# mbitsnbites/himg

Hardware: AMD Instinct MI355X
Metric: Mpixels/s encode+decode, 4K RGBA q=50 (higher is better)
Workload: dtype u8/i16/i32 integer

## Files before the change

himg_amd/csrc/himg_dev.h:

```cpp
#ifndef HIMG_DEV_H_
#define HIMG_DEV_H_

#include <hip/hip_runtime.h>
#include <stdint.h>

#include "search_step.h"

namespace himg_dev {

constexpr int kNumSym = 261;
constexpr int kHistStride = 264;
constexpr int kLresSpan = 16384;
constexpr int kIterSyms = 4096;
constexpr int kTreeStride = 384;
constexpr int kMaxCodeLen = 32;
constexpr int kHeadLen = 175;

struct Geom {
  int W, H, C, stride;
  int rows, cols, mrows, mcols;
  int chan_size, lres_size;
  int row_block;
  int ycbcr;
  int lres_spans;
  int use_blocks;
  int fix_t2;
  int lres_serial;
  int max_sub;
  int lead_bits;
  int prefetch_rows;
  int count_wave;
  int wide_q;
  int emit_rows;
  int front;
  int row_tokens;
  long long frame_bytes;
  long long fres_size;
};

struct EncWs {
  uint8_t *avg, *low;        size_t plane_stride;
  uint8_t *lres_sym;         size_t lres_stride;
  uint8_t *fres_sym;         size_t fres_stride;
  uint32_t *hist;
  uint32_t *span_hist_l;
  uint32_t *span_hist_f;
  uint32_t *lres_trail;
  uint64_t *codes;
  uint32_t *lens;
  uint8_t *tree;
  uint32_t *tree_nbytes;
  uint64_t *span_bit0;
  uint32_t *span_bits;
  int32_t *status;
  uint16_t *tok;
  uint32_t *tok_cnt;
  int tok_seg, tok_nseg, tok_cap;
};

constexpr uint32_t kTokRunMark = 0x0100u;
constexpr int kTokMaxRun = 255;
constexpr int kTokIter = 2048;
constexpr int kTokRunPiece = 16662;
constexpr int kTokStage = 1152;
inline int tok_slots_beyond(int zeros_max) { return 5 + 3 * (zeros_max / kTokRunPiece); }
inline int tok_seg_pad(int row_block) {
  const int pad = (tok_slots_beyond(row_block) + 7) & ~7;
  return pad > 64 ? pad : 64;
}
inline int tok_stage_need(int row_block, int seg) {
  const int alone = 1024 + tok_slots_beyond(row_block);
  const int carried = 7 + 1024 + tok_slots_beyond(seg < row_block ? seg : row_block);
  return alone > carried ? alone : carried;
}

struct StaticChunks {
  uint8_t head[176];
  uint8_t mid[272];
  int mid_len;
};

struct ShiftTables {
  uint8_t s[2][64];
};

struct LresTables {
  int16_t tab[128];
  uint8_t code[512];
};

struct QualTab {
// ... 228 lines not shown
```

himg_amd/csrc/himg_hip.hip:

```cpp
#include "himg_hip.h"

#include <hip/hip_runtime.h>

#include <cmath>
#include <cstdio>
#include <cstdlib>
#include <cstring>
#include <string>
#include <vector>

#include "himg_dev.h"
#include "himg_tables.h"

using namespace himg_dev;

namespace himg_dev {

struct Profiler {
  bool enabled = false;
  struct Rec { const char *name; hipEvent_t a, b; };
  std::vector<Rec> pending;
  struct Acc { std::string name; double ms = 0; int n = 0; };
  std::vector<Acc> acc;
  const char *cur = nullptr;
// ... 28 lines not shown
  hipEvent_t b;
  hipEventCreate(&b);
  hipEventRecord(b, s);
  p->pending.push_back({p->cur, p->cur_a, b});
}

}

namespace {

struct DevBuf {
  void *p = nullptr;
  size_t cap = 0;
  bool reserve(size_t n) {
    if (n <= cap) return true;
    if (p) hipFree(p);
    p = nullptr;
    cap = 0;
    if (hipMalloc(&p, n) != hipSuccess) return false;
    cap = n;
    return true;
  }
  void release() {
    if (p) hipFree(p);
    p = nullptr;
    cap = 0;
  }
};

size_t round_up(size_t x, size_t a) { return (x + a - 1) / a * a; }

struct HostResult {
  uint32_t size;
  int32_t status;
  int32_t quality;
  uint64_t sse;
};
struct PipeMeta {
  HostResult res[2];
  uint32_t dec_size[2];
};

}

struct himg_hip_ctx {
  int device = 0;
  std::string err;
  Profiler prof;
  hipStream_t last_stream = nullptr;
  HostOpts opts;
  int fix_t2 = 0;
  int max_sub = 4096;
  int lead_bits = 128;
  int lres_serial = 0;
  int prefetch_rows = 1;
  int count_wave = -1, emit_rows = -1;
  int row_tokens = -1;
  int front = -1;
  DecStreams dstr;
  hipStream_t side_enc = nullptr;
  hipEvent_t ev_fork_e = nullptr, ev_join_e = nullptr;

  DevBuf fmap_lut;
  size_t host_bytes = 0;
  struct Pipe {
    bool ready = false;
    hipStream_t s_in = nullptr, s_comp = nullptr, s_out = nullptr;
    hipEvent_t ev_in[2] = {nullptr, nullptr}, ev_k[2] = {nullptr, nullptr}, ev_out[2] = {nullptr, nullptr};
    DevBuf in[2], out[2], meta[2];
    PipeMeta *h_meta = nullptr;
  } pipe;

  DevBuf e_planes, e_lres, e_fres, e_small, e_spanhist, e_tok, e_tokx;
  DevBuf e_qtab, e_search;
  DevBuf e_stab, e_rec;
  bool qtab_ready = false;
  Geom enc_geom{};
  EncWs enc_ws{};
  int enc_batch = 0;
  bool enc_valid = false;

  DevBuf d_frames, d_nodes, d_grp, d_gyc, d_sub, d_lane, d_rows, d_lres, d_fres, d_planes, d_sizes, d_stats, d_spec;
  Geom dec_geom{};
  DecWs dec_ws{};
  int dec_batch = 0;
  bool dec_valid = false;
  hipEvent_t ev_range[HIMG_MAX_WALK_RANGES] = {};
  int n_ranges = 0;
  struct HeadToken {
    bool valid = false;
    int w = 0, h = 0, c = 0;
    const void *packed = nullptr;
    uint32_t size = 0;
    void *stream = nullptr;
  } head;

  DevBuf h_in, h_out, h_result, h_status, h_index;
  uint32_t *hp_index = nullptr;
  size_t hp_index_cap = 0;

  struct SizeRing {
    static constexpr int kSlots = 4;
    uint32_t *h[kSlots] = {nullptr, nullptr, nullptr, nullptr};
    size_t cap[kSlots] = {0, 0, 0, 0};
    hipEvent_t ev[kSlots] = {nullptr, nullptr, nullptr, nullptr};
    bool busy[kSlots] = {false, false, false, false};
    int next = 0;
  } sizes_ring;

  struct {
    bool valid = false;
    Geom g{};
    StaticChunks sc{};
    ShiftTables st{};
    LresTables lt{};
    int r0 = 0, r1 = 0;
  } shard;
};

static int fail(himg_hip_ctx *ctx, int code, const char *what, hipError_t e = hipSuccess) {
  if (ctx) {
    ctx->err = what;
    if (e != hipSuccess) { ctx->err += ": "; ctx->err += hipGetErrorString(e); }
  }
  return code;
}

#define HIP_TRY(ctx, expr)                                                  \
  do {                                                                      \
    hipError_t e_ = (expr);                                                 \
    if (e_ != hipSuccess) return fail(ctx, HIMG_ERR_HIP, #expr, e_);        \
  } while (0)

static bool make_geom(int width, int height, int pixel_stride, int num_channels, int use_ycbcr,
                      Geom *g) {
  if (width < 1 || height < 1 || num_channels < 1 || num_channels > 4 ||
      pixel_stride < num_channels)
    return false;
  g->W = width; g->H = height; g->C = num_channels; g->stride = pixel_stride;
  g->rows = (height + 7) >> 3; g->cols = (width + 7) >> 3;
  g->mrows = (g->rows + 15) / 16; g->mcols = (g->cols + 15) / 16;
  g->chan_size = g->mrows * g->mcols + g->rows * g->cols;
  const long long lres = (long long)g->chan_size * num_channels;
  const long long fres = (long long)g->rows * g->cols * 64 * num_channels;
  if (fres > 0x7fffffffLL || (long long)width * height * pixel_stride > 0x7fffffffLL) return false;
  g->lres_size = (int)lres;
  g->row_block = g->cols * num_channels * 64;
  g->ycbcr = (use_ycbcr && num_channels >= 3) ? 1 : 0;
  g->lres_spans = (g->lres_size + kLresSpan - 1) / kLresSpan;
  g->use_blocks = g->rows > 1 ? 1 : 0;
  g->fix_t2 = 0;
  g->max_sub = 4096;
  g->lead_bits = 128;
  g->lres_serial = 0;
  g->count_wave = g->emit_rows = g->row_tokens = g->front = -1;
  g->wide_q = 0;
  g->prefetch_rows = 1;
  g->frame_bytes = (long long)width * height * pixel_stride;
  g->fres_size = fres;
  return true;
}

static void apply_settings(const himg_hip_ctx *ctx, Geom *g) {
  g->fix_t2 = ctx->fix_t2;
  g->max_sub = ctx->max_sub;
  g->lead_bits = ctx->lead_bits;
  g->lres_serial = ctx->lres_serial;
  g->prefetch_rows = ctx->prefetch_rows;
  g->count_wave = ctx->count_wave;
  g->emit_rows = ctx->emit_rows;
  g->row_tokens = ctx->row_tokens;
  g->front = ctx->front;
}

extern "C" size_t himg_hip_max_packed_size(int width, int height, int num_channels) {
  Geom g;
  if (!make_geom(width, height, num_channels, num_channels, 1, &g)) return 0;
  size_t n = 12 + 19 + 136 + 8 + 72 + 188 + 8;
  n += (size_t)g.lres_size + kTreeStride;
  n += (size_t)g.fres_size + kTreeStride + 4u * (size_t)g.rows;
  return round_up(n + 64, 256);
}

extern "C" int himg_hip_create(int device, himg_hip_ctx **out) {
  if (!out) return HIMG_ERR_ARG;
  *out = nullptr;
  int count = 0;
  if (hipGetDeviceCount(&count) != hipSuccess || count < 1) return HIMG_ERR_HIP;
  if (device < 0 || device >= count) return HIMG_ERR_ARG;
  if (hipSetDevice(device) != hipSuccess) return HIMG_ERR_HIP;
  himg_hip_ctx *ctx = new himg_hip_ctx();
  ctx->device = device;
  HostOpts &o = ctx->opts;
  if (const char *e = std::getenv("HIMG_FORCE_UNFUSED")) o.allow_fused = !(e[0] == '1');
  if (const char *e = std::getenv("HIMG_WALK_SEGS")) o.walk_segs = atoi(e);
  if (const char *e = std::getenv("HIMG_SIDE_STREAM")) o.use_side = !(e[0] == '0');
  if (const char *e = std::getenv("HIMG_PERSIST_ROWS")) o.persist_rows = atoi(e);
  if (const char *e = std::getenv("HIMG_PREFETCH_ROWS")) ctx->prefetch_rows = atoi(e);
  if (const char *e = std::getenv("HIMG_FIX_T2")) ctx->fix_t2 = e[0] == '1';
  if (const char *e = std::getenv("HIMG_FORCE_LRES_SERIAL")) ctx->lres_serial = e[0] == '1';
  if (const char *e = std::getenv("HIMG_MAX_SUB_BITS")) {
    const int v = std::atoi(e);
    if (v >= 128 && v <= 4096 && v % 32 == 0) ctx->max_sub = v;
  }
  if (const char *e = std::getenv("HIMG_COUNT_WAVE")) ctx->count_wave = atoi(e) ? 1 : 0;
  if (const char *e = std::getenv("HIMG_EMIT_ROWS")) ctx->emit_rows = atoi(e) ? 1 : 0;
  if (const char *e = std::getenv("HIMG_ROW_TOKENS")) ctx->row_tokens = atoi(e) ? 1 : 0;
  if (const char *e = std::getenv("HIMG_FRONT")) ctx->front = atoi(e) ? 1 : 0;
  if (const char *e = std::getenv("HIMG_LEAD_BITS")) {
    const int v = std::atoi(e);
    if (v >= 0 && v <= 4096) ctx->lead_bits = v;
  }
  int n_cu = 0;
  if (hipDeviceGetAttribute(&n_cu, hipDeviceAttributeMultiprocessorCount, device) == hipSuccess && n_cu > 0) o.n_cu = n_cu;
  if (himg_dev::enc_set_kernel_attrs() != hipSuccess || himg_dev::dec_set_kernel_attrs() != hipSuccess) {
    delete ctx;
    return HIMG_ERR_HIP;
  }
  std::vector<uint8_t> lut(32769);
  int16_t fmap[128];
  himg_tables_fullres_map(fmap);
  for (int a = 0; a <= 32767; ++a) lut[a] = himg_tables_map_to_8bit(fmap, a);
  lut[32768] = (uint8_t)(0u - himg_tables_map_to_8bit(fmap, -32768));
  if (!ctx->fmap_lut.reserve(round_up(lut.size(), 256)) ||
      hipMemcpy(ctx->fmap_lut.p, lut.data(), lut.size(), hipMemcpyHostToDevice) != hipSuccess) {
    delete ctx;
    return HIMG_ERR_HIP;
  }
  int prio_least = 0, prio_greatest = 0;
  (void)hipDeviceGetStreamPriorityRange(&prio_least, &prio_greatest);
  bool ev_ok = true;
  for (int k = 0; k < kWalkSegs; ++k)
    ev_ok = ev_ok && hipEventCreateWithFlags(&ctx->dstr.ev_walk[k], hipEventDisableTiming) == hipSuccess &&
            hipEventCreateWithFlags(&ctx->dstr.ev_cnt[k], hipEventDisableTiming) == hipSuccess &&
            hipEventCreateWithFlags(&ctx->dstr.ev_win[k], hipEventDisableTiming) == hipSuccess;
  if (!ev_ok || hipStreamCreateWithPriority(&ctx->dstr.side, hipStreamNonBlocking, prio_least) != hipSuccess ||
      hipStreamCreateWithPriority(&ctx->dstr.side2, hipStreamNonBlocking, prio_least) != hipSuccess ||
      hipEventCreateWithFlags(&ctx->dstr.ev_fork, hipEventDisableTiming) != hipSuccess ||
      hipStreamCreateWithFlags(&ctx->side_enc, hipStreamNonBlocking) != hipSuccess ||
      hipEventCreateWithFlags(&ctx->ev_fork_e, hipEventDisableTiming) != hipSuccess ||
      hipEventCreateWithFlags(&ctx->ev_join_e, hipEventDisableTiming) != hipSuccess) {
    himg_hip_destroy(ctx);
    return HIMG_ERR_HIP;
  }
  ctx->dstr.side3 = ctx->side_enc;
  *out = ctx;
  return HIMG_OK;
}

extern "C" void himg_hip_destroy(himg_hip_ctx *ctx) {
  if (!ctx) return;
  hipSetDevice(ctx->device);
  hipDeviceSynchronize();
// ... 223 lines not shown
  const size_t plane = round_up((size_t)g.C * g.rows * g.cols, 256);
  const size_t lres = round_up((size_t)g.lres_size + 16, 256);
  const size_t fres = round_up((size_t)g.fres_size + 16, 256);
  if (head_only) {
    const size_t nst = 2 * (size_t)batch - 1;
    if (!ctx->d_frames.reserve(sizeof(DecFrame) * batch) || !ctx->d_nodes.reserve(nst * (2 * kNumSym) * 4) ||
        !ctx->d_grp.reserve(nst * (1u << kLutBits) * 8) || !ctx->d_gyc.reserve(nst * (1u << kLutBits) * 4) ||
        !ctx->d_sub.reserve(nst * kSubEntries * 8) || !ctx->d_lres.reserve(lres * batch) ||
        !ctx->d_planes.reserve(plane * batch) || !ctx->d_sizes.reserve((size_t)batch * 8) ||
        !ctx->d_stats.reserve(((size_t)batch * (g.rows + 1) * 8 + (size_t)batch * 4) * 4))
      return fail(ctx, HIMG_ERR_HIP, "decoder workspace allocation failed");
  } else if (!ctx->d_frames.reserve(sizeof(DecFrame) * batch) ||
      !ctx->d_nodes.reserve((size_t)batch * 2 * (2 * kNumSym) * 4) ||
      !ctx->d_grp.reserve((size_t)batch * 2 * (1u << kLutBits) * 8) ||
      !ctx->d_gyc.reserve((size_t)batch * 2 * (1u << kLutBits) * 4) ||
      !ctx->d_sub.reserve((size_t)batch * 2 * kSubEntries * 8) ||
      !ctx->d_lane.reserve((size_t)batch * g.rows * (2 * kDecThreads + himg_dev::kRecHdr + (region || himg_dev::dec_rows_fit_lds(g) ? 0 : 6 * kDecThreads)) * 4) ||
      !ctx->d_rows.reserve((size_t)batch * g.rows * 4 * 2) || !ctx->d_lres.reserve(lres * batch) ||
      (!region && !ctx->d_fres.reserve(fres * batch)) || !ctx->d_planes.reserve(plane * batch) ||
      !ctx->d_sizes.reserve((size_t)batch * 20) ||
      !ctx->d_stats.reserve(((size_t)batch * (g.rows + 1) * 8 + (size_t)batch * 4 + (size_t)batch * g.rows * 8) * 4))
    return fail(ctx, HIMG_ERR_HIP, "decoder workspace allocation failed");
  w.frames = (DecFrame *)ctx->d_frames.p;
  w.nodes = (uint32_t *)ctx->d_nodes.p;
  w.grp = (uint2 *)ctx->d_grp.p;
  w.gyc = (uint32_t *)ctx->d_gyc.p;
  w.sub = (uint2 *)ctx->d_sub.p;
  w.lane_start = head_only ? nullptr : (uint32_t *)ctx->d_lane.p;
  w.lane_off = head_only ? nullptr : w.lane_start + (size_t)batch * g.rows * kDecThreads;
  w.lane_q = (head_only || region || himg_dev::dec_rows_fit_lds(g)) ? nullptr : w.lane_off + (size_t)batch * g.rows * (kDecThreads + himg_dev::kRecHdr);
  w.row_off = head_only ? nullptr : (uint32_t *)ctx->d_rows.p;
  w.row_len = head_only ? nullptr : w.row_off + (size_t)batch * g.rows;
  w.lres_sym = (uint8_t *)ctx->d_lres.p; w.lres_stride = lres;
  w.fres_sym = (head_only || region) ? nullptr : (uint8_t *)ctx->d_fres.p; w.fres_stride = (head_only || region) ? 0 : fres;
  w.low = (uint8_t *)ctx->d_planes.p; w.plane_stride = plane;
  w.stats = (uint32_t *)ctx->d_stats.p;
  w.parse_stats = w.stats + (size_t)batch * (g.rows + 1) * 8;
  w.rc_stats = head_only ? nullptr : w.parse_stats + (size_t)batch * 4;
  {
    const size_t max_bits = 8ull * ((size_t)g.lres_size + kTreeStride);
    const size_t cb = (size_t)kDecThreads * kLresSubBits;
    int nch = (int)((max_bits + cb - 1) / cb);
    if (nch > 1024) nch = 1024;
    w.lres_chunks = nch;
    size_t off = 0;
    auto carve = [&](size_t bytes) { size_t o = off; off += round_up(bytes, 256); return o; };
    const size_t o_ss = carve((size_t)batch * nch * kDecThreads * 4);
    const size_t o_sc = carve((size_t)batch * nch * kDecThreads * 4);
    const size_t o_se = carve((size_t)batch * nch * 8);
    const size_t o_st = carve((size_t)batch * nch * 8);
    const size_t o_sp = carve((size_t)batch * nch * kDecThreads * 4);
    const size_t o_fe = carve((size_t)batch * nch * 8);
    const size_t o_vb = carve((size_t)batch * nch * 8);
    const size_t o_ok = carve((size_t)batch * 4);
    const size_t o_eb = carve((size_t)batch * 8);
    const size_t o_mm = carve((size_t)batch * nch * kDecThreads * 4 * himg_dev::kLresMemoWords);
    if (!ctx->d_spec.reserve(off)) return fail(ctx, HIMG_ERR_HIP, "decoder workspace allocation failed");
    uint8_t *b = (uint8_t *)ctx->d_spec.p;
    w.spec_start = (uint32_t *)(b + o_ss); w.spec_cnt = (uint32_t *)(b + o_sc);
    w.spec_end = (uint64_t *)(b + o_se); w.spec_tot = (uint64_t *)(b + o_st);
    w.spec_endpos = (uint32_t *)(b + o_sp); w.fix_end = (uint64_t *)(b + o_fe);
    w.ver_base = (uint64_t *)(b + o_vb); w.ver_ok = (int32_t *)(b + o_ok);
    w.lres_endbit = (uint64_t *)(b + o_eb);
    w.spec_memo = (uint32_t *)(b + o_mm);
  }
  ctx->dec_geom = g;
  ctx->dec_batch = batch;
  ctx->dec_valid = true;
  return HIMG_OK;
}

static std::string format_message(int32_t st) {
  static const char *kStage[] = {"", "Not a RIFF HIMG file.\n", "Error decoding header.\n",
                                 "Error decoding low-res mapping function.\n",
                                 "Error decoding low-res data.\n",
                                 "Error decoding quantization configuration.\n",
                                 "Error decoding full-res mapping function.\n",
                                 "Error decoding full-res data.\n"};
  std::string m;
  if (st & 0x100) m += "Error: Invalid Huffman data.\n";
  const int stage = (st >> 4) & 7;
  m += kStage[stage];
  return m;
}

static int status_to_code(int32_t st) {
  st &= 15;
  switch (st) {
    case 0: return HIMG_OK;
    case 1: return HIMG_ERR_ARG;
    case 3: return HIMG_ERR_UNSUPPORTED;
    case 4: return HIMG_ERR_FORMAT;
    case 5: return HIMG_ERR_CAPACITY;
    default: return HIMG_ERR_HIP;
  }
}

static int status_error(himg_hip_ctx *ctx, int32_t st, const char *what = "device decode reported an error") {
  const int code = status_to_code(st);
  if (code == HIMG_ERR_FORMAT) ctx->err = format_message(st);
  else fail(ctx, code, what);
  return code;
}

static int decode_args(himg_hip_ctx *ctx, int width, int height, int num_channels, int batch, DecWsKind kind,
                       const void *d_packed, const void *d_out, const size_t *in_stride, const char *bad, Geom *g) {
  if (!make_geom(width, height, num_channels, num_channels, 1, g)) return fail(ctx, HIMG_ERR_ARG, "bad geometry");
// ... 1971 lines not shown
```

himg_amd/csrc/kernels_dec.hip:

```cpp
#include "himg_dev.h"
#include "loop_counts.h"

#include <cstdlib>
#include <type_traits>

namespace himg_dev {

__device__ static constexpr uint8_t kScanD[64] = {
    0,  1,  9,  8,  16, 17, 18, 10, 2,  3,  11, 19, 27, 26, 25, 24,
    32, 33, 34, 35, 36, 28, 20, 12, 4,  5,  13, 21, 29, 37, 45, 44,
    43, 42, 41, 40, 48, 49, 50, 51, 52, 53, 54, 46, 38, 30, 22, 14,
    6,  7,  15, 23, 31, 39, 47, 55, 63, 62, 61, 60, 59, 58, 57, 56};

__device__ static constexpr uint8_t kInvScanD[64] = {
    0, 1, 8, 9, 24, 25, 48, 49, 3, 2, 7, 10, 23, 26, 47, 50, 4, 5, 6, 11, 22, 27, 46, 51, 15, 14, 13, 12, 21, 28, 45, 52, 16, 17, 18, 19, 20, 29, 44, 53, 35, 34, 33, 32, 31, 30, 43, 54, 36, 37, 38, 39, 40, 41, 42, 55, 63, 62, 61, 60, 59, 58, 57, 56};

constexpr int kStGeom = 1, kStUnsupported = 3, kStFormat = 4;
__device__ __host__ constexpr int fmt_err(int stage, int huff) { return kStFormat | (stage << 4) | (huff << 8); }
constexpr int kMaxDepth = 32;
constexpr int kMaxNodes = 2 * kNumSym - 1;
constexpr int kMaxSlow = 128;

__device__ __forceinline__ int clamp255d(int x) { return x < 0 ? 0 : (x > 255 ? 255 : x); }

// ... 1369 lines not shown
  if (end_bp != ~0u) sh->endbit = (unsigned long long)(end_bp - rel0);
  __syncthreads();
  const long long c_t1 = clock64();
  int bad = sh->err;
  if (pl.tot < out_size) bad = 1;
  const unsigned long long E = sh->endbit;
  if (!bad && !(E <= P1 && E + 8 > P1 && E > 0)) bad = 1;
  if (tid == 0 && stats) {
    stats[0] = 1; stats[1] = pl.rounds;
    stats[4] = 0; stats[5] = (uint32_t)((c_t1 - c_t0) >> 4);
    stats[6] = pay_len; stats[7] = out_size;
  }
  return bad;
}

__device__ __attribute__((noinline)) int decode_stream_fused_cold(const uint8_t *p, uint32_t stream_size,
                                                                  uint32_t pay_off, uint32_t pay_len, uint32_t out_size,
                                                                  const uint32_t *grp_lds, const uint32_t *nd_lds,
                                                                  StreamShared *sh, uint8_t *lds_out, uint32_t *stats,
                                                                  uint32_t max_sub, uint32_t lead_bits) {
  GrpTables tb;
  tb.grp = reinterpret_cast<const uint2 *>(grp_lds); tb.gx = nullptr; tb.gy = nullptr; tb.nd = nd_lds;
  return decode_stream<true, false, true>(p, stream_size, pay_off, pay_len, out_size, tb, sh, lds_out, nullptr, nullptr,
                                          stats, max_sub, lead_bits);
}

__device__ __forceinline__ void load_dec_tables(const DecWs &ws, const DecFrame *df, int f, int strm,
                                                LdsTables *T) {
  const uint32_t *nodes = ws.nodes + ((size_t)f * 2 + strm) * (kMaxNodes + 1);
  const int nn = min(df->s[strm].num_nodes, kMaxNodes + 1);
  for (int k = threadIdx.x; k < nn; k += kDecThreads) T->nd[k] = nodes[k];
  const uint4 *gg = reinterpret_cast<const uint4 *>(ws.grp + ((size_t)f * 2 + strm) * (1u << kLutBits));
  for (int k = threadIdx.x; k < (1 << kLutBits) / 2; k += kDecThreads)
    reinterpret_cast<uint4 *>(T->grp)[k] = gg[k];
  const uint4 *gs = reinterpret_cast<const uint4 *>(ws.sub + ((size_t)f * 2 + strm) * kSubEntries);
  for (int k = threadIdx.x; k < kSubEntries / 2; k += kDecThreads)
    reinterpret_cast<uint4 *>(T->grp + (1 << kLutBits))[k] = gs[k];
}

__global__ __launch_bounds__(kDecThreads) void k_dec_huff(Geom g, DecWs ws, const uint8_t *packed,
                                                          size_t in_stride, const uint32_t *sizes,
                                                          int first_block, int lres_fallback_only,
                                                          int use_row_count) {
  __shared__ uint32_t win[kWinBytes / 4 + 1];
  __shared__ LdsTables T;
  __shared__ StreamShared sh;

  const int blk = blockIdx.x + first_block, f = blockIdx.y;
  DecFrame *df = ws.frames + f;
  if (threadIdx.x == 0) sh.flag = df->status;
  __syncthreads();
  if (sh.flag) return;
  const int strm = blk == 0 ? 0 : 1;
  if (strm == 0 && lres_fallback_only && ws.ver_ok[f]) return;
  const uint8_t *p = packed + (size_t)f * in_stride;
  uint32_t pay_off, pay_len, out_size;
  uint8_t *out;
  const uint32_t *pre_start = nullptr, *pre_off = nullptr;
  if (strm == 0) {
    pay_off = df->s[0].payload_off;
    pay_len = df->s[0].chunk_end - pay_off;
    out_size = (uint32_t)g.lres_size;
    out = ws.lres_sym + (size_t)f * ws.lres_stride;
  } else {
    const int r = blk - 1;
    pay_off = ws.row_off[(size_t)f * g.rows + r];
    pay_len = ws.row_len[(size_t)f * g.rows + r];
    out_size = (uint32_t)g.row_block;
    out = ws.fres_sym + (size_t)f * ws.fres_stride + (size_t)r * g.row_block;
    if (use_row_count) {
      pre_start = ws.lane_start + ((size_t)f * g.rows + r) * kDecThreads;
      pre_off = ws.lane_off + ((size_t)f * g.rows + r) * (kDecThreads + kRecHdr);
      if (use_row_count == 2 && pre_off[kDecThreads + 2] != 0) return;
    }
  }
  load_dec_tables(ws, df, f, strm, &T);
  __syncthreads();
  const GrpTables tb = tables_of(&T);
  const int bad = decode_stream<false>(p, sizes[f], pay_off, pay_len, out_size, tb, &sh, nullptr, win,
                                       out, ws.stats + ((size_t)f * (g.rows + 1) + blk) * 8,
                                       (uint32_t)g.max_sub, (uint32_t)g.lead_bits, pre_start, pre_off);
  if (bad && threadIdx.x == 0) atomicMax(&df->status, fmt_err(strm == 0 ? 4 : 7, 1));
}

constexpr int kLresChunkBits = kDecThreads * kLresSubBits;

constexpr int kLresPayWords = kDecThreads * kLresSubBits / 32 + 8;
constexpr int kLresMemo = kLresMemoWords;
template <bool FIX>
__device__ __forceinline__ void lres_chain_body(const Geom &g, const DecWs &ws, const uint8_t *p, uint32_t stream_size,
                                const DecFrame *df, int f, int k, const GrpTables &tb, StreamShared *sh,
                                uint32_t *s_pay) {
  const int tid = threadIdx.x;
  const uint32_t pay_off = df->s[0].payload_off;
  const unsigned long long P1 = 8ull * (df->s[0].chunk_end - pay_off);
  const unsigned long long cur = (unsigned long long)k * kLresChunkBits;
  const size_t slot = (size_t)f * ws.lres_chunks + k;
  uint64_t *end_out = FIX ? ws.fix_end : ws.spec_end;
  GReader gr;
  const uint32_t rel0 = gr.attach(p, stream_size, 8ull * pay_off + cur);
  LReader rd;
  stage_payload(gr, s_pay, (uint32_t)kLresPayWords);
  __syncthreads();
  rd.w = (const __attribute__((address_space(3))) uint32_t *)s_pay;
  rd.jmax = kLresPayWords - 1;
  const unsigned long long rem = P1 - cur;
  const uint32_t rel_end = rel0 + (uint32_t)(rem < (unsigned long long)kLresChunkBits ? rem : kLresChunkBits);
// ... 24 lines not shown
      if (m != ~0u) { memo[3 * e] = my_b0 + (m & 63u); memo[3 * e + 1] = lim + ((m >> 6) & 63u); memo[3 * e + 2] = m >> 12; }
    }
  }
  const long long c_in = clock64();
  lean_fixpoint<false, LReader, kLresMemo>(rd, tb, sh, first, active, lim, &start, &endpos, &cnt, &rounds, FIX,
                                           (uint32_t)g.lead_bits, nullptr, nullptr, memo);
  const long long c_fix = clock64() - c_in;
  if (!FIX) {
#pragma unroll
    for (int e = 0; e < kLresMemo; ++e) {
      const uint32_t ds = memo[3 * e] - my_b0, de = memo[3 * e + 1] - lim;
      gm[e] = (memo[3 * e] == ~0u || tid == 0 || ds > 46u || de > 46u || memo[3 * e + 2] >= (1u << 20))
                  ? ~0u : (ds | (de << 6) | (memo[3 * e + 2] << 12));
    }
  }
  unsigned long long tot;
  block_scan_u64(cnt, sh->sm64, &tot);
  ws.spec_start[slot * kDecThreads + tid] = start - rel0;
  ws.spec_endpos[slot * kDecThreads + tid] = endpos - rel0;
  ws.spec_cnt[slot * kDecThreads + tid] = cnt;
  if (tid == last_active) { end_out[slot] = cur + (endpos - rel0); ws.spec_tot[slot] = tot; }
  if (tid == 0) {
    uint32_t *st = ws.stats + ((size_t)f * (g.rows + 1)) * 8;
    atomicAdd(&st[FIX ? 2 : 0], 1u);
    atomicAdd(&st[FIX ? 3 : 1], rounds);
    atomicMax(&st[FIX ? 5 : 4], rounds);
    atomicMax(&st[FIX ? 7 : 6], (uint32_t)(c_fix >> 4));
  }
}

__global__ __launch_bounds__(kDecThreads) void k_lres_spec(Geom g, DecWs ws, const uint8_t *packed,
                                                           size_t in_stride, const uint32_t *sizes) {
  __shared__ LdsTables T;
  __shared__ StreamShared sh;
  __shared__ __attribute__((aligned(16))) uint32_t s_pay[kLresPayWords];
  const int k = blockIdx.x, f = blockIdx.y, tid = threadIdx.x;
  DecFrame *df = ws.frames + f;
  if (tid == 0) sh.flag = df->status;
  __syncthreads();
  if (sh.flag) return;
  const unsigned long long P1 = 8ull * (df->s[0].chunk_end - df->s[0].payload_off);
  const unsigned long long cur = (unsigned long long)k * kLresChunkBits;
  const size_t slot = (size_t)f * ws.lres_chunks + k;
  if (cur >= P1) {
    if (tid == 0) { ws.spec_end[slot] = cur; ws.spec_tot[slot] = 0; }
    return;
  }
  load_dec_tables(ws, df, f, 0, &T);
  __syncthreads();
  const GrpTables tb = tables_of(&T);
  lres_chain_body<false>(g, ws, packed + (size_t)f * in_stride, sizes[f], df, f, k, tb, &sh, s_pay);
}

__global__ __launch_bounds__(kDecThreads) void k_lres_fix(Geom g, DecWs ws, const uint8_t *packed,
                                                          size_t in_stride, const uint32_t *sizes) {
  __shared__ LdsTables T;
  __shared__ StreamShared sh;
  __shared__ uint8_t s_pending[kDecThreads];
  __shared__ int s_bad;
  __shared__ __attribute__((aligned(16))) uint32_t s_pay[kLresPayWords];
  const int f = blockIdx.x, k = threadIdx.x;
  DecFrame *df = ws.frames + f;
  if (k == 0) { ws.ver_ok[f] = 0; ws.lres_endbit[f] = ~0ull; s_bad = 0; sh.flag = df->status; }
  s_pending[k] = 0;
  __syncthreads();
  if (sh.flag) return;
  const uint32_t pay_off = df->s[0].payload_off;
  const unsigned long long P1 = 8ull * (df->s[0].chunk_end - pay_off);
  const int nact = (int)((P1 + kLresChunkBits - 1) / kLresChunkBits);
  if (nact > ws.lres_chunks || nact > kDecThreads) return;
  load_dec_tables(ws, df, f, 0, &T);
  __syncthreads();
  const GrpTables tb = tables_of(&T);
  const uint8_t *p = packed + (size_t)f * in_stride;
  const size_t slot = (size_t)f * ws.lres_chunks + k;
  const unsigned long long cur = (unsigned long long)k * kLresChunkBits;
  if (k == 0) {
    ws.fix_end[slot] = ws.spec_end[slot];
  } else if (k < nact) {
    const unsigned long long T = ws.spec_end[slot - 1];
    bool settled = false;
    if (T >= cur && T < cur + kLresSubBits) {
      GReader rd;
      const uint32_t rel0 = rd.attach(p, sizes[f], 8ull * pay_off + cur);
      const unsigned long long rem = P1 - cur;
      uint32_t lim = rel0 + kLresSubBits;
      const uint32_t rel_end = rel0 + (uint32_t)(rem < (unsigned long long)kLresChunkBits ? rem : kLresChunkBits);
      if (lim > rel_end) lim = rel_end;
      uint32_t pos, c;
      lean_count(rd, tb, rel0 + (uint32_t)(T - cur), lim, &pos, &c);
      if (pos - rel0 == ws.spec_endpos[slot * kDecThreads]) {
        const unsigned long long oldc = ws.spec_cnt[slot * kDecThreads];
        ws.spec_start[slot * kDecThreads] = (uint32_t)(T - cur);
        ws.spec_cnt[slot * kDecThreads] = c;
        ws.spec_tot[slot] = ws.spec_tot[slot] - oldc + c;
        ws.fix_end[slot] = ws.spec_end[slot];
        settled = true;
        atomicAdd(&ws.stats[((size_t)f * (g.rows + 1)) * 8 + 2], 1u);
      }
    }
    if (!settled) s_pending[k] = 1;
  }
  __syncthreads();
  for (int q = 1; q < nact; ++q) {
    if (!s_pending[q]) continue;
    lres_chain_body<true>(g, ws, p, sizes[f], df, f, q, tb, &sh, s_pay);
    __syncthreads();
  }
  __threadfence_block();
  __syncthreads();
  unsigned long long ntot = 0;
  if (k < nact) {
    ntot = ws.spec_tot[slot];
    if (k + 1 < nact && ws.fix_end[slot] != ws.spec_end[slot]) s_bad = 1;
  }
  unsigned long long tot;
  const unsigned long long base = block_scan_u64(ntot, sh.sm64, &tot);
  if (k < nact) ws.ver_base[slot] = base;
  __syncthreads();
  if (k == 0) ws.ver_ok[f] = (s_bad || g.lres_serial) ? 0 : 1;
}

__global__ __launch_bounds__(kDecThreads) void k_lres_write(Geom g, DecWs ws, const uint8_t *packed,
                                                            size_t in_stride, const uint32_t *sizes) {
  __shared__ LdsTables T;
  __shared__ StreamShared sh;
  const int k = blockIdx.x, f = blockIdx.y, tid = threadIdx.x;
  DecFrame *df = ws.frames + f;
  const size_t slot = (size_t)f * ws.lres_chunks + k;
  const unsigned long long O0 = ws.ver_base[slot];
  const uint32_t start_rel = ws.spec_start[slot * kDecThreads + tid];
  const unsigned long long cnt = ws.spec_cnt[slot * kDecThreads + tid];
  if (tid == 0) sh.flag = df->status ? 1 : (ws.ver_ok[f] ? 0 : 2);
  load_dec_tables(ws, df, f, 0, &T);
  __syncthreads();
  if (sh.flag == 1) return;
  if (sh.flag == 2) {
    if (k != 0) return;
    const GrpTables tb0 = tables_of(&T);
    const uint32_t po = df->s[0].payload_off;
    const int bad = decode_stream<false, true>(packed + (size_t)f * in_stride, sizes[f], po, df->s[0].chunk_end - po,
                                               (uint32_t)g.lres_size, tb0, &sh, nullptr, nullptr,
                                               ws.lres_sym + (size_t)f * ws.lres_stride,
                                               ws.stats + ((size_t)f * (g.rows + 1)) * 8, (uint32_t)g.max_sub,
                                               (uint32_t)g.lead_bits);
    if (bad && tid == 0) atomicMax(&df->status, fmt_err(4, 1));
    return;
  }
  const uint32_t pay_off = df->s[0].payload_off;
  const unsigned long long P1 = 8ull * (df->s[0].chunk_end - pay_off);
  const unsigned long long cur = (unsigned long long)k * kLresChunkBits;
  if (cur >= P1) return;
  const uint32_t out_size = (uint32_t)g.lres_size;
  if (O0 >= out_size) return;
  if (tid == 0) { sh.err = 0; sh.endbit = ~0ull; }
  const GrpTables tb = tables_of(&T);
  GReader rd;
  const uint32_t rel0 = rd.attach(packed + (size_t)f * in_stride, sizes[f], 8ull * pay_off + cur);
  const unsigned long long rem = P1 - cur;
  const uint32_t rel_end = rel0 + (uint32_t)(rem < (unsigned long long)kLresChunkBits ? rem : kLresChunkBits);
  uint32_t lim = rel0 + (tid + 1) * kLresSubBits;
  if (lim > rel_end) lim = rel_end;
  const uint32_t start = rel0 + start_rel;
  __syncthreads();
  unsigned long long tot;
  const unsigned long long off = block_scan_u64(cnt, sh.sm64, &tot);
  const unsigned long long opl = O0 + off;
  const bool exact = !(opl + cnt < out_size) && opl < out_size;
  lean_write_global(rd, tb, &sh, start, lim, opl, exact, out_size, cur, rel0,
                    ws.lres_sym + (size_t)f * ws.lres_stride, exact ? opl : opl + cnt);
  __syncthreads();
  if (tid == 0) {
    if (sh.err) atomicMax(&df->status, fmt_err(4, 1));
    if (sh.endbit != ~0ull) ws.lres_endbit[f] = sh.endbit;
  }
}

__global__ void k_lres_finish(DecWs ws, int batch) {
  const int f = blockIdx.x * blockDim.x + threadIdx.x;
  if (f >= batch) return;
  DecFrame *df = ws.frames + f;
  if (df->status || !ws.ver_ok[f]) return;
  const unsigned long long P1 = 8ull * (df->s[0].chunk_end - df->s[0].payload_off);
  const unsigned long long E = ws.lres_endbit[f];
  if (!(E != ~0ull && E <= P1 && E + 8 > P1 && E > 0)) atomicMax(&df->status, fmt_err(4, 1));
}

__device__ __forceinline__ int predict_d(int s1, int s2, int s3, int p) {
  switch (p) {
    default:
    case 0: return clamp255d((3 * (s2 + s3) - 2 * s1 + 2) >> 2);
    case 1: return s2;
    case 2: return s3;
    case 3: return (s2 + s3 + 1) >> 1;
    case 4: return clamp255d(s2 + s3 - s1);
  }
}

__device__ __forceinline__ void wave_lds_sync() {
  __builtin_amdgcn_fence(__ATOMIC_RELEASE, "wavefront");
  __builtin_amdgcn_wave_barrier();
  __builtin_amdgcn_fence(__ATOMIC_ACQUIRE, "wavefront");
}

constexpr int kUnpredWaves = 4;
__global__ __launch_bounds__(64 * kUnpredWaves) void k_lres_unpredict(Geom g, DecWs ws) {
  __shared__ uint8_t rec_s[kUnpredWaves][4][17][18];
  __shared__ uint8_t dl_s[kUnpredWaves][4][16][16];
  __shared__ int16_t s_lmap[128];
  __shared__ int s_status;
  const int lane = threadIdx.x & 63, wv = threadIdx.x >> 6, b = lane >> 4, dv = lane & 15;
  uint8_t (*rec)[17][18] = rec_s[wv];
  uint8_t (*dl)[16][16] = dl_s[wv];
  const int mu = (blockIdx.x * kUnpredWaves + wv) * 4 + b, mv = blockIdx.y;
  const int f = blockIdx.z / g.C, c = blockIdx.z % g.C;
  const DecFrame *df = ws.frames + f;
  if (threadIdx.x == 0) s_status = df->status;
  if (threadIdx.x < 128) s_lmap[threadIdx.x] = df->lmap[threadIdx.x];
  const uint8_t *in = ws.lres_sym + (size_t)f * ws.lres_stride + (size_t)c * g.chan_size;
  uint8_t *m = ws.low + (size_t)f * ws.plane_stride + (size_t)c * g.rows * g.cols;
  const bool live = mu < g.mcols;
  const int u0 = mu * 16, v0 = mv * 16;
  const int bw = live ? min(16, g.cols - u0) : 0, bh = min(16, g.rows - v0);
  const int pc = live ? (int)in[mv * g.mcols + mu] + 2 : 0;
  const uint8_t *src = in + g.mrows * g.mcols + (size_t)v0 * g.cols + (size_t)bh * u0;
  if (dv < bh) {
#pragma unroll
    for (int k = 0; k < 16; ++k)
      if (k < bw) dl[b][dv][k] = src[dv * bw + k];
  }
  __syncthreads();
  if (s_status) return;
  const bool row_live = dv < bh, up_ok = dv > 0;
  uint8_t *rrow = &rec[b][dv + 1][1];
  const uint8_t *urow = &rec[b][dv][1];
// ... 2314 lines not shown
  if (e != hipSuccess) return e;
  hipFuncAttributes fa;
  e = hipFuncGetAttributes(&fa, reinterpret_cast<const void *>(&k_dec_region));
  if (e == hipSuccess)
    e = hipFuncSetAttribute(reinterpret_cast<const void *>(&k_dec_region), hipFuncAttributeMaxDynamicSharedMemorySize,
                            (int)(kLdsMax - fa.sharedSizeBytes));
  if (e == hipSuccess) e = hipFuncGetAttributes(&fa, reinterpret_cast<const void *>(&k_dec_region_t));
  if (e == hipSuccess)
    e = hipFuncSetAttribute(reinterpret_cast<const void *>(&k_dec_region_t), hipFuncAttributeMaxDynamicSharedMemorySize,
                            (int)(kLdsMax - fa.sharedSizeBytes));
  if (e == hipSuccess) e = hipFuncGetAttributes(&fa, reinterpret_cast<const void *>(&k_dec_region_p));
  if (e == hipSuccess)
    e = hipFuncSetAttribute(reinterpret_cast<const void *>(&k_dec_region_p), hipFuncAttributeMaxDynamicSharedMemorySize,
                            (int)(kLdsMax - fa.sharedSizeBytes));
  const void *scaled[] = {reinterpret_cast<const void *>(&k_dec_scaled<4, true>), reinterpret_cast<const void *>(&k_dec_scaled<2, true>),
                          reinterpret_cast<const void *>(&k_dec_scaled<4, false>), reinterpret_cast<const void *>(&k_dec_scaled<2, false>),
                          reinterpret_cast<const void *>(&k_dec_scaled_region<4>), reinterpret_cast<const void *>(&k_dec_scaled_region<2>)};
  for (const void *k : scaled) {
    if (e == hipSuccess) e = hipFuncGetAttributes(&fa, k);
    if (e == hipSuccess)
      e = hipFuncSetAttribute(k, hipFuncAttributeMaxDynamicSharedMemorySize, (int)(kLdsMax - fa.sharedSizeBytes));
  }
  return e;
}

int region_strip_tiles(const Geom &g) {
  const uint32_t fixed = region_layout(g.C, 0).total - region_layout(g.C, 0).seg * 64u * (uint32_t)g.C;
  const uint32_t seg = (kLdsMax - 1024u - fixed) / (64u * (uint32_t)g.C) & ~3u;
  return (int)(seg - 8u);
}

int scaled_strip_tiles(const Geom &g, int scale_log2) {
  const uint32_t nseg = (scale_log2 == 1 ? 16u : 4u) * (uint32_t)g.C;
  const RegionLayout L0 = scale_log2 == 1 ? scaled_layout<4>(g.C, 0) : scaled_layout<2>(g.C, 0);
  const uint32_t fixed = L0.total - L0.seg * nseg;
  const uint32_t seg = (kLdsMax - 1024u - fixed) / nseg & ~3u;
  return (int)(seg - 8u);
}

void launch_rowwalk_only(const Geom &g, const DecWs &ws, const uint8_t *d_packed, size_t in_stride,
                         const uint32_t *d_sizes, hipStream_t stream) {
  hipLaunchKernelGGL(k_dec_rowwalk, dim3(1), dim3(64), 0, stream, g, ws, d_packed, in_stride, d_sizes, 0x7fffffff, 0);
}

void launch_rowwalk_range(const Geom &g, const DecWs &ws, const uint8_t *d_packed, size_t in_stride,
                          const uint32_t *d_sizes, int row_end, bool resume, hipStream_t stream) {
  hipLaunchKernelGGL(k_dec_rowwalk, dim3(1), dim3(64), 0, stream, g, ws, d_packed, in_stride, d_sizes, row_end, resume ? 1 : 0);
}

static void launch_lres_chain(const Geom &g, const DecWs &ws, int batch, const uint8_t *d_packed, size_t in_stride,
                              const uint32_t *d_sizes, hipStream_t stream, Profiler *prof) {
  HIMG_LAUNCH(k_lres_spec, dim3(ws.lres_chunks, batch), dim3(kDecThreads), g, ws, d_packed, in_stride, d_sizes);
  HIMG_LAUNCH(k_lres_fix, dim3(batch), dim3(kDecThreads), g, ws, d_packed, in_stride, d_sizes);
  HIMG_LAUNCH(k_lres_write, dim3(ws.lres_chunks, batch), dim3(kDecThreads), g, ws, d_packed,
              in_stride, d_sizes);
  HIMG_LAUNCH(k_lres_finish, dim3((batch + 63) / 64), dim3(64), ws, batch);
  HIMG_LAUNCH(k_lres_unpredict, dim3((g.mcols + 4 * kUnpredWaves - 1) / (4 * kUnpredWaves), g.mrows, batch * g.C),
              dim3(64 * kUnpredWaves), g, ws);
}

static void launch_zero(const Geom &g, const DecWs &ws, int batch, hipStream_t stream, Profiler *prof) {
  const uint32_t n16 = (uint32_t)(((size_t)batch * ws.lres_stride + 15) / 16);
  const uint32_t ns = (uint32_t)((size_t)batch * (g.rows + 1) * 8), nr = ws.rc_stats ? (uint32_t)((size_t)batch * g.rows * 8) : 0u;
  prof_begin(prof, "memset", stream);
  hipLaunchKernelGGL(k_dec_zero, dim3((n16 + 256 * 4 - 1) / (256 * 4)), dim3(256), 0, stream,
                     reinterpret_cast<uint4 *>(ws.lres_sym), n16, ws.stats, ns, ws.rc_stats, nr);
  prof_end(prof, stream);
}

struct CountRule { bool wave; int rpc; Geom g; };
static CountRule count_rule(const Geom &g, long long all_rows, bool one_record) {
  CountRule c = {g.count_wave >= 0 ? g.count_wave != 0 : all_rows >= 8192,
                 all_rows <= 512 ? 1 : all_rows <= 1024 ? 2 : kRowsPerCount, g};
  if (one_record) c.g.max_sub = 0x7fffffff;
  return c;
}

void launch_preview(const Geom &g, const DecWs &ws, int batch, const uint8_t *d_packed, size_t in_stride,
                    const uint32_t *d_sizes, uint32_t *d_head_sizes, uint8_t *d_out, int32_t *d_status,
                    hipStream_t stream, Profiler *prof) {
  launch_zero(g, ws, batch, stream, prof);
  HIMG_LAUNCH(k_dec_parse_head, dim3(batch), dim3(kParseThreads), g, ws, d_packed, in_stride, d_sizes, d_head_sizes);
  launch_lres_chain(g, ws, batch, d_packed, in_stride, d_head_sizes, stream, prof);
  const uint32_t npix = (uint32_t)g.rows * (uint32_t)g.cols;
  HIMG_LAUNCH(k_lres_preview, dim3((npix + 1023u) / 1024u, batch), dim3(256), g, ws, d_out);
  HIMG_LAUNCH(k_dec_status, dim3((batch + 63) / 64), dim3(64), ws, d_status, batch);
}

struct WindowExtents { int nrows = 0, ntiles = 0; long long all_rows = 0; bool stop_early = false; };
static WindowExtents window_extents(const Geom &g, int batch, const int32_t *h_org, int S, int w, int h) {
  WindowExtents e;
  const int F = 8 / S;
  for (int f = 0; f < batch; ++f) {
    const int x = h_org[2 * f] / F, y = h_org[2 * f + 1] / F;
    const int r0 = y / S, r1 = (y + h + S - 1) / S, nt = (x + w + S - 1) / S - x / S;
    e.nrows = r1 - r0 > e.nrows ? r1 - r0 : e.nrows;
    e.ntiles = nt > e.ntiles ? nt : e.ntiles;
    e.stop_early |= r1 < g.rows;
    e.all_rows += r1 - r0;
  }
  return e;
}

void launch_region(const Geom &g, const DecWs &ws_in, int batch, const uint8_t *d_packed, size_t in_stride,
                   const uint32_t *d_sizes, const uint32_t *d_row_index, const int32_t *h_org, const int32_t *d_org,
                   int scale_log2, int w, int h, uint8_t *d_out, int32_t *d_status, hipStream_t stream, Profiler *prof,
                   const DecStreams *ds, const TensDesc *tens, const DstDesc *dst) {
  DecWs ws = ws_in;
// ... 344 lines not shown
```

Before: 100,200.

## Split rare slow paths out of lres fix and write kernels

The LRES fix kernel now handles only the fast settled case. If any chunk is still unresolved it marks the chunk pending and defers the serial chain re-decode to a new k_lres_fix_warm kernel. The serial fallback decode moves out of k_lres_write into k_lres_write_serial. The slimmed fast-path kernels drop large shared buffers and gain launch-bounds occupancy hints, aiming for lower register and LDS pressure and better occupancy. In exchange, each decode launches two extra kernels that usually exit early, and ver_ok doubles in size to carry a per-frame warm flag.

New measurement: 100,400 (median of 6 runs). Within noise of the previous version (+0.2%).

```diff
diff --git a/himg_amd/csrc/himg_dev.h b/himg_amd/csrc/himg_dev.h
--- a/himg_amd/csrc/himg_dev.h
+++ b/himg_amd/csrc/himg_dev.h
@@ -25,7 +25,7 @@
   int lres_spans;
   int use_blocks;
   int fix_t2;
-  int lres_serial;
+  int lres_force;
   int max_sub;
   int lead_bits;
   int prefetch_rows;
@@ -37,6 +37,8 @@
   long long frame_bytes;
   long long fres_size;
 };
+
+constexpr int kLresForceSerial = 1, kLresForceWarm = 2;
 
 struct EncWs {
   uint8_t *avg, *low;        size_t plane_stride;
diff --git a/himg_amd/csrc/himg_hip.hip b/himg_amd/csrc/himg_hip.hip
--- a/himg_amd/csrc/himg_hip.hip
+++ b/himg_amd/csrc/himg_hip.hip
@@ -104,7 +104,7 @@
   int fix_t2 = 0;
   int max_sub = 4096;
   int lead_bits = 128;
-  int lres_serial = 0;
+  int lres_force = 0;
   int prefetch_rows = 1;
   int count_wave = -1, emit_rows = -1;
   int row_tokens = -1;
@@ -204,7 +204,7 @@
   g->fix_t2 = 0;
   g->max_sub = 4096;
   g->lead_bits = 128;
-  g->lres_serial = 0;
+  g->lres_force = 0;
   g->count_wave = g->emit_rows = g->row_tokens = g->front = -1;
   g->wide_q = 0;
   g->prefetch_rows = 1;
@@ -217,7 +217,7 @@
   g->fix_t2 = ctx->fix_t2;
   g->max_sub = ctx->max_sub;
   g->lead_bits = ctx->lead_bits;
-  g->lres_serial = ctx->lres_serial;
+  g->lres_force = ctx->lres_force;
   g->prefetch_rows = ctx->prefetch_rows;
   g->count_wave = ctx->count_wave;
   g->emit_rows = ctx->emit_rows;
@@ -250,7 +250,8 @@
   if (const char *e = std::getenv("HIMG_PERSIST_ROWS")) o.persist_rows = atoi(e);
   if (const char *e = std::getenv("HIMG_PREFETCH_ROWS")) ctx->prefetch_rows = atoi(e);
   if (const char *e = std::getenv("HIMG_FIX_T2")) ctx->fix_t2 = e[0] == '1';
-  if (const char *e = std::getenv("HIMG_FORCE_LRES_SERIAL")) ctx->lres_serial = e[0] == '1';
+  if (const char *e = std::getenv("HIMG_FORCE_LRES_SERIAL")) ctx->lres_force |= e[0] == '1' ? himg_dev::kLresForceSerial : 0;
+  if (const char *e = std::getenv("HIMG_FORCE_LRES_WARM")) ctx->lres_force |= e[0] == '1' ? himg_dev::kLresForceWarm : 0;
   if (const char *e = std::getenv("HIMG_MAX_SUB_BITS")) {
     const int v = std::atoi(e);
     if (v >= 128 && v <= 4096 && v % 32 == 0) ctx->max_sub = v;
@@ -580,7 +581,7 @@
     const size_t o_sp = carve((size_t)batch * nch * kDecThreads * 4);
     const size_t o_fe = carve((size_t)batch * nch * 8);
     const size_t o_vb = carve((size_t)batch * nch * 8);
-    const size_t o_ok = carve((size_t)batch * 4);
+    const size_t o_ok = carve((size_t)batch * 2 * 4);
     const size_t o_eb = carve((size_t)batch * 8);
     const size_t o_mm = carve((size_t)batch * nch * kDecThreads * 4 * himg_dev::kLresMemoWords);
     if (!ctx->d_spec.reserve(off)) return fail(ctx, HIMG_ERR_HIP, "decoder workspace allocation failed");
diff --git a/himg_amd/csrc/kernels_dec.hip b/himg_amd/csrc/kernels_dec.hip
--- a/himg_amd/csrc/kernels_dec.hip
+++ b/himg_amd/csrc/kernels_dec.hip
@@ -1445,7 +1445,7 @@
   __syncthreads();
   if (sh.flag) return;
   const int strm = blk == 0 ? 0 : 1;
-  if (strm == 0 && lres_fallback_only && ws.ver_ok[f]) return;
+  if (strm == 0 && lres_fallback_only && ws.ver_ok[2 * f]) return;
   const uint8_t *p = packed + (size_t)f * in_stride;
   uint32_t pay_off, pay_len, out_size;
   uint8_t *out;
@@ -1576,17 +1576,38 @@
   lres_chain_body<false>(g, ws, packed + (size_t)f * in_stride, sizes[f], df, f, k, tb, &sh, s_pay);
 }
 
-__global__ __launch_bounds__(kDecThreads) void k_lres_fix(Geom g, DecWs ws, const uint8_t *packed,
-                                                          size_t in_stride, const uint32_t *sizes) {
+constexpr unsigned long long kLresFixPending = ~1ull;
+__device__ __forceinline__ int32_t &lres_verified(const DecWs &ws, int f) { return ws.ver_ok[2 * f]; }
+__device__ __forceinline__ int32_t &lres_warm(const DecWs &ws, int f) { return ws.ver_ok[2 * f + 1]; }
+
+__device__ __forceinline__ void lres_verify(const Geom &g, const DecWs &ws, int f, int nact, StreamShared *sh, int *s_bad) {
+  const int k = threadIdx.x;
+  const size_t slot = (size_t)f * ws.lres_chunks + k;
+  __threadfence_block();
+  __syncthreads();
+  unsigned long long ntot = 0;
+  if (k < nact) {
+    ntot = ws.spec_tot[slot];
+    if (k + 1 < nact && ws.fix_end[slot] != ws.spec_end[slot]) *s_bad = 1;
+  }
+  unsigned long long tot;
+  const unsigned long long base = block_scan_u64(ntot, sh->sm64, &tot);
+  if (k < nact) ws.ver_base[slot] = base;
+  __syncthreads();
+  if (k == 0) lres_verified(ws, f) = (*s_bad || (g.lres_force & kLresForceSerial)) ? 0 : 1;
+}
+
+__global__ __launch_bounds__(kDecThreads, 7) void k_lres_fix(Geom g, DecWs ws, const uint8_t *packed,
+                                                             size_t in_stride, const uint32_t *sizes) {
   __shared__ LdsTables T;
   __shared__ StreamShared sh;
-  __shared__ uint8_t s_pending[kDecThreads];
-  __shared__ int s_bad;
-  __shared__ __attribute__((aligned(16))) uint32_t s_pay[kLresPayWords];
+  __shared__ int s_bad, s_pending;
   const int f = blockIdx.x, k = threadIdx.x;
   DecFrame *df = ws.frames + f;
-  if (k == 0) { ws.ver_ok[f] = 0; ws.lres_endbit[f] = ~0ull; s_bad = 0; sh.flag = df->status; }
-  s_pending[k] = 0;
+  if (k == 0) {
+    lres_verified(ws, f) = 0; lres_warm(ws, f) = 0; ws.lres_endbit[f] = ~0ull;
+    s_bad = 0; s_pending = 0; sh.flag = df->status;
+  }
   __syncthreads();
   if (sh.flag) return;
   const uint32_t pay_off = df->s[0].payload_off;
@@ -1604,7 +1625,7 @@
   } else if (k < nact) {
     const unsigned long long T = ws.spec_end[slot - 1];
     bool settled = false;
-    if (T >= cur && T < cur + kLresSubBits) {
+    if (T >= cur && T < cur + kLresSubBits && !(g.lres_force & kLresForceWarm)) {
       GReader rd;
       const uint32_t rel0 = rd.attach(p, sizes[f], 8ull * pay_off + cur);
       const unsigned long long rem = P1 - cur;
@@ -1623,30 +1644,45 @@
         atomicAdd(&ws.stats[((size_t)f * (g.rows + 1)) * 8 + 2], 1u);
       }
     }
-    if (!settled) s_pending[k] = 1;
-  }
-  __syncthreads();
+    if (!settled) { ws.fix_end[slot] = kLresFixPending; s_pending = 1; }
+  }
+  __syncthreads();
+  if (s_pending) {
+    if (k == 0) lres_warm(ws, f) = 1;
+    return;
+  }
+  lres_verify(g, ws, f, nact, &sh, &s_bad);
+}
+
+__global__ __launch_bounds__(kDecThreads) void k_lres_fix_warm(Geom g, DecWs ws, const uint8_t *packed,
+                                                               size_t in_stride, const uint32_t *sizes) {
+  __shared__ LdsTables T;
+  __shared__ StreamShared sh;
+  __shared__ uint8_t s_pending[kDecThreads];
+  __shared__ int s_bad;
+  __shared__ __attribute__((aligned(16))) uint32_t s_pay[kLresPayWords];
+  const int f = blockIdx.x, k = threadIdx.x;
+  DecFrame *df = ws.frames + f;
+  if (k == 0) { s_bad = 0; sh.flag = lres_warm(ws, f); }
+  __syncthreads();
+  if (!sh.flag) return;
+  const unsigned long long P1 = 8ull * (df->s[0].chunk_end - df->s[0].payload_off);
+  const int nact = (int)((P1 + kLresChunkBits - 1) / kLresChunkBits);
+  s_pending[k] = k >= 1 && k < nact && ws.fix_end[(size_t)f * ws.lres_chunks + k] == kLresFixPending;
+  load_dec_tables(ws, df, f, 0, &T);
+  __syncthreads();
+  const GrpTables tb = tables_of(&T);
+  const uint8_t *p = packed + (size_t)f * in_stride;
   for (int q = 1; q < nact; ++q) {
     if (!s_pending[q]) continue;
     lres_chain_body<true>(g, ws, p, sizes[f], df, f, q, tb, &sh, s_pay);
     __syncthreads();
   }
-  __threadfence_block();
-  __syncthreads();
-  unsigned long long ntot = 0;
-  if (k < nact) {
-    ntot = ws.spec_tot[slot];
-    if (k + 1 < nact && ws.fix_end[slot] != ws.spec_end[slot]) s_bad = 1;
-  }
-  unsigned long long tot;
-  const unsigned long long base = block_scan_u64(ntot, sh.sm64, &tot);
-  if (k < nact) ws.ver_base[slot] = base;
-  __syncthreads();
-  if (k == 0) ws.ver_ok[f] = (s_bad || g.lres_serial) ? 0 : 1;
-}
-
-__global__ __launch_bounds__(kDecThreads) void k_lres_write(Geom g, DecWs ws, const uint8_t *packed,
-                                                            size_t in_stride, const uint32_t *sizes) {
+  lres_verify(g, ws, f, nact, &sh, &s_bad);
+}
+
+__global__ __launch_bounds__(kDecThreads, 7) void k_lres_write(Geom g, DecWs ws, const uint8_t *packed,
+                                                               size_t in_stride, const uint32_t *sizes) {
   __shared__ LdsTables T;
   __shared__ StreamShared sh;
   const int k = blockIdx.x, f = blockIdx.y, tid = threadIdx.x;
@@ -1655,22 +1691,10 @@
   const unsigned long long O0 = ws.ver_base[slot];
   const uint32_t start_rel = ws.spec_start[slot * kDecThreads + tid];
   const unsigned long long cnt = ws.spec_cnt[slot * kDecThreads + tid];
-  if (tid == 0) sh.flag = df->status ? 1 : (ws.ver_ok[f] ? 0 : 2);
+  if (tid == 0) sh.flag = df->status || !lres_verified(ws, f);
   load_dec_tables(ws, df, f, 0, &T);
   __syncthreads();
-  if (sh.flag == 1) return;
-  if (sh.flag == 2) {
-    if (k != 0) return;
-    const GrpTables tb0 = tables_of(&T);
-    const uint32_t po = df->s[0].payload_off;
-    const int bad = decode_stream<false, true>(packed + (size_t)f * in_stride, sizes[f], po, df->s[0].chunk_end - po,
-                                               (uint32_t)g.lres_size, tb0, &sh, nullptr, nullptr,
-                                               ws.lres_sym + (size_t)f * ws.lres_stride,
-                                               ws.stats + ((size_t)f * (g.rows + 1)) * 8, (uint32_t)g.max_sub,
-                                               (uint32_t)g.lead_bits);
-    if (bad && tid == 0) atomicMax(&df->status, fmt_err(4, 1));
-    return;
-  }
+  if (sh.flag) return;
   const uint32_t pay_off = df->s[0].payload_off;
   const unsigned long long P1 = 8ull * (df->s[0].chunk_end - pay_off);
   const unsigned long long cur = (unsigned long long)k * kLresChunkBits;
@@ -1700,11 +1724,32 @@
   }
 }
 
+__global__ __launch_bounds__(kDecThreads) void k_lres_write_serial(Geom g, DecWs ws, const uint8_t *packed,
+                                                                   size_t in_stride, const uint32_t *sizes) {
+  __shared__ LdsTables T;
+  __shared__ StreamShared sh;
+  const int f = blockIdx.x, tid = threadIdx.x;
+  DecFrame *df = ws.frames + f;
+  if (tid == 0) sh.flag = !df->status && !lres_verified(ws, f);
+  __syncthreads();
+  if (!sh.flag) return;
+  load_dec_tables(ws, df, f, 0, &T);
+  __syncthreads();
+  const GrpTables tb0 = tables_of(&T);
+  const uint32_t po = df->s[0].payload_off;
+  const int bad = decode_stream<false, true>(packed + (size_t)f * in_stride, sizes[f], po, df->s[0].chunk_end - po,
+                                             (uint32_t)g.lres_size, tb0, &sh, nullptr, nullptr,
+                                             ws.lres_sym + (size_t)f * ws.lres_stride,
+                                             ws.stats + ((size_t)f * (g.rows + 1)) * 8, (uint32_t)g.max_sub,
+                                             (uint32_t)g.lead_bits);
+  if (bad && tid == 0) atomicMax(&df->status, fmt_err(4, 1));
+}
+
 __global__ void k_lres_finish(DecWs ws, int batch) {
   const int f = blockIdx.x * blockDim.x + threadIdx.x;
   if (f >= batch) return;
   DecFrame *df = ws.frames + f;
-  if (df->status || !ws.ver_ok[f]) return;
+  if (df->status || !lres_verified(ws, f)) return;
   const unsigned long long P1 = 8ull * (df->s[0].chunk_end - df->s[0].payload_off);
   const unsigned long long E = ws.lres_endbit[f];
   if (!(E != ~0ull && E <= P1 && E + 8 > P1 && E > 0)) atomicMax(&df->status, fmt_err(4, 1));
@@ -4125,8 +4170,10 @@
                               const uint32_t *d_sizes, hipStream_t stream, Profiler *prof) {
   HIMG_LAUNCH(k_lres_spec, dim3(ws.lres_chunks, batch), dim3(kDecThreads), g, ws, d_packed, in_stride, d_sizes);
   HIMG_LAUNCH(k_lres_fix, dim3(batch), dim3(kDecThreads), g, ws, d_packed, in_stride, d_sizes);
+  HIMG_LAUNCH(k_lres_fix_warm, dim3(batch), dim3(kDecThreads), g, ws, d_packed, in_stride, d_sizes);
   HIMG_LAUNCH(k_lres_write, dim3(ws.lres_chunks, batch), dim3(kDecThreads), g, ws, d_packed,
               in_stride, d_sizes);
+  HIMG_LAUNCH(k_lres_write_serial, dim3(batch), dim3(kDecThreads), g, ws, d_packed, in_stride, d_sizes);
   HIMG_LAUNCH(k_lres_finish, dim3((batch + 63) / 64), dim3(64), ws, batch);
   HIMG_LAUNCH(k_lres_unpredict, dim3((g.mcols + 4 * kUnpredWaves - 1) / (4 * kUnpredWaves), g.mrows, batch * g.C),
               dim3(64 * kUnpredWaves), g, ws);
```
